# yz-cnsdqz/PSI-release

Hardware: AMD Instinct MI355X
Metric: fitting iters/sec (SMPL-X+SDF+Chamfer), PROX-E batch=32 (higher is better)
Workload: dtype f32

## Files before the change

### psi-release_amd/csrc/fit.hip

```cpp
#include "psi_internal.h"
#ifdef PSI_HEAD_STOPS
__device__ int psi_dbg_sstop;
#define PSI_SSTOP(k) do { if (psi_dbg_sstop == (k)) return; } while (0)
__device__ int psi_dbg_pstop;
#define PSI_PSTOP(k) do { if (psi_dbg_pstop == (k)) asm volatile("s_endpgm"); } while (0)
#define PSI_TRACE(lo, hi) PsiBlockTrace trace_((lo), (hi))
__device__ unsigned long long psi_dbg_tl[4 * 8192];
struct PsiBlockTrace {
    unsigned long long t0;
    int kind;
    int sel_lo, sel_hi;
    __device__ PsiBlockTrace(int lo = 9, int hi = 10) : t0(wall_clock64()), kind(0), sel_lo(lo), sel_hi(hi) {}
    __device__ ~PsiBlockTrace()
    {
        const unsigned bid = blockIdx.y * gridDim.x + blockIdx.x;
        if (psi_dbg_sstop < sel_lo || psi_dbg_sstop > sel_hi || threadIdx.x != 0 || bid >= 8192) return;
        unsigned long long *o = psi_dbg_tl + 4 * (size_t)bid;
        o[0] = t0;
        o[1] = wall_clock64();
        o[2] = (unsigned long long)__builtin_amdgcn_s_getreg((31 << 11) | 4) | ((unsigned long long)__builtin_amdgcn_s_getreg((31 << 11) | 20) << 32);
        o[3] = (unsigned long long)kind;
    }
};
extern "C" int psi_dbg_timeline(unsigned long long *out, int nblocks)
// ... 48 lines not shown
    const float *scene, *sdf, *gmin, *gmax;
    const float *sdf_brick;
    const float *Wct;
    float *x, *xhr, *cam, *adam_m, *adam_v;
    int *step;
    float *h1, *h2, *o6, *betas20, *pose, *transl, *verts, *og, *gq, *fpart, *penpart, *recpart, *vppart;
    float *cverts;
    float *g_betas, *g_pose, *g_transl, *g_rot;
    unsigned long long *hx_o6, *hx_gh1;
    unsigned *hx_epoch;
    int *hx_err;
    int hc;
#ifdef PSI_HEAD_STOPS
    int stop_h, stop_t;
#define HSTOP(k) do { if (f.stop_h == (k)) return; } while (0)
#define TSTOP(k) do { if (f.stop_t == (k)) return; } while (0)
#else
#define HSTOP(k)
#define TSTOP(k)
#endif
    int *nn_hint;
    float *history;
    int max_hist;
    int fused_bwd, ncp, ncp3;
    float *glc, *gvpc, *vpc;
    float *gtc_part;
#ifndef PSI_GV_SLOTS
#define PSI_GV_SLOTS 1024
#endif
    static_assert(PSI_GV_SLOTS >= 128, "one slot per body and class at least: fused_bwd runs batches up to 128 (merged_scene)");
    unsigned *gvbits;
    int gv_sps;
    const float *dirs_ch;
    const float *WTt_c;
    float *gA_part, *gfeat_part;
    float *spb;
    int nsv, nsv_c, nsn_m, nsn_c, spm, spc;
};

__device__ __forceinline__ float leaky(float v, float slope) { return v > 0.0f ? v : v * slope; }

__device__ __forceinline__ void gs_forward(const float *x6, float *R)
{
    float a1[3] = {x6[0], x6[2], x6[4]}, a2[3] = {x6[1], x6[3], x6[5]};
    float n1 = fmaxf(sqrtf(a1[0] * a1[0] + a1[1] * a1[1] + a1[2] * a1[2]), 1e-12f);
    float b1[3] = {a1[0] / n1, a1[1] / n1, a1[2] / n1};
    float d = b1[0] * a2[0] + b1[1] * a2[1] + b1[2] * a2[2];
    float u[3] = {a2[0] - d * b1[0], a2[1] - d * b1[1], a2[2] - d * b1[2]};
    float n2 = fmaxf(sqrtf(u[0] * u[0] + u[1] * u[1] + u[2] * u[2]), 1e-12f);
    float b2[3] = {u[0] / n2, u[1] / n2, u[2] / n2};
    float b3[3] = {b1[1] * b2[2] - b1[2] * b2[1], b1[2] * b2[0] - b1[0] * b2[2], b1[0] * b2[1] - b1[1] * b2[0]};
    for (int r = 0; r < 3; r++) {
        R[r * 3 + 0] = b1[r];
        R[r * 3 + 1] = b2[r];
        R[r * 3 + 2] = b3[r];
    }
}

__device__ __forceinline__ void gs_backward(const float *x6, const float *gR, float *g6)
{
    float a1[3] = {x6[0], x6[2], x6[4]}, a2[3] = {x6[1], x6[3], x6[5]};
    float n1 = fmaxf(sqrtf(a1[0] * a1[0] + a1[1] * a1[1] + a1[2] * a1[2]), 1e-12f);
    float b1[3] = {a1[0] / n1, a1[1] / n1, a1[2] / n1};
    float d = b1[0] * a2[0] + b1[1] * a2[1] + b1[2] * a2[2];
    float u[3] = {a2[0] - d * b1[0], a2[1] - d * b1[1], a2[2] - d * b1[2]};
    float n2 = fmaxf(sqrtf(u[0] * u[0] + u[1] * u[1] + u[2] * u[2]), 1e-12f);
    float b2[3] = {u[0] / n2, u[1] / n2, u[2] / n2};
// ... 654 lines not shown
            a2 += p[(size_t)(i + 2 * nt) * stride];
            a3 += p[(size_t)(i + 3 * nt) * stride];
        }
        for (; i < n; i += nt) a0 += p[(size_t)i * stride];
        return block_sum((a0 + a1) + (a2 + a3), red);
    };
    const float s_rec = total(f.recpart, f.B, 1);
    const float s_vp = total(f.vppart, f.B, 1);
    const float s_f = total(f.fpart, f.B * f.nfp, 1);
    const float s_pen = total(f.penpart, f.B * f.nsdfblk, 2);
    const float n_pen = total(f.penpart + 1, f.B * f.nsdfblk, 2);
    if (t == 0) {
        stats[0] = s_rec; stats[1] = s_vp; stats[2] = s_f; stats[3] = s_pen; stats[4] = n_pen; stats[5] = 0.0f;
        *f.step += 1;
    }
}

template <int MT>
__global__ __launch_bounds__(256) __attribute__((amdgpu_waves_per_eu(2, 2))) void fit_bwd_joint_kernel(
    FitDev f, LbsDev m, const float *__restrict__ g_vp, const float *__restrict__ gl, const float *__restrict__ v_posed, int n_ska, int n_blend,
    int kgroups, int nbody, float *__restrict__ stats)
{
    constexpr int SMEM_B = psi_blend_bwd_h_smem_f4<(MT + 1) / 2>();
    __shared__ f4 smem[SMEM_B > SKA_SMEM_F4 ? SMEM_B : SKA_SMEM_F4];
    const int bid = blockIdx.x;
#ifdef PSI_HEAD_STOPS
    PsiBlockTrace trace(11, 11);
    trace.kind = bid < n_ska ? (bid % (f.nsv + f.nsv_c) < f.nsv ? 0 : 1) : (bid < n_ska + n_blend ? 2 : 4);
#endif
    if (bid < n_ska) {
        const int nsl = f.nsv + f.nsv_c, sl = bid % nsl, b0 = (bid / nsl) * nbody;
        float *part = f.gA_part + (size_t)sl * f.B * PSI_JP * 16;
        if (sl < f.nsv) {
            const PsiSkaSlice o = {m.WTt + (size_t)sl * 4 * PSI_JP * 64, gl + (size_t)sl * 768, v_posed + (size_t)sl * 768, (size_t)m.Npad, part};
            skin_bwd_A_dispatch(o, f.B, b0, nbody, smem);
        } else {
            const int c = sl - f.nsv;
            const PsiSkaSlice o = {f.WTt_c + (size_t)c * 4 * PSI_JP * 64, f.glc + (size_t)c * 768, f.vpc + (size_t)c * 768, (size_t)f.ncp3, part};
            skin_bwd_A_dispatch(o, f.B, b0, nbody, smem);
        }
    } else if (bid < n_ska + n_blend) {
        int kg, slice, bg;
        psi_blend_bwd_place(bid - n_ska, kgroups, f.nsn_m + f.nsn_c, kg, slice, bg);
#ifdef PSI_HEAD_STOPS
        trace.kind = slice < f.nsn_m ? 2 : 3;
#endif
        float *part = f.gfeat_part + (size_t)slice * f.B * m.Kpad;
        const float dsc_inv = m.dirs_unscale * PSI_FEAT_SCALE;
        if (slice < f.nsn_m) {
            const PsiBlendBwdColsH o = {m.dirs_bh, g_vp, (size_t)m.Npad, m.Kpad, m.Npad / 16, f.gvbits, f.gv_sps, dsc_inv};
            blend_bwd_h_body<(MT + 1) / 2>(o, f.B, slice * f.spm, (slice + 1) * f.spm, part, kg, bg, smem);
        } else {
            const int c = slice - f.nsn_m;
            const PsiBlendBwdColsH o = {f.dirs_ch, f.gvpc, (size_t)f.ncp3, m.Kpad, f.ncp3 / 16, f.gvbits + PSI_GV_SLOTS, f.gv_sps, dsc_inv};
            blend_bwd_h_body<(MT + 1) / 2>(o, f.B, c * f.spc, (c + 1) * f.spc, part, kg, bg, smem);
        }
    } else {
        fit_stats_body(f, stats);
    }
}

__global__ __launch_bounds__(256) void fit_reduce_kernel(FitDev f, PsiLbsView lv, const float *__restrict__ stats)
{
    const int B = f.B, Kpad = lv.m.Kpad;
    const long nA = (long)B * PSI_JP * 16, nF = (long)B * Kpad, nT = (long)B * 4;
    const long t = (long)blockIdx.x * 256 + threadIdx.x;
    const long i = t / PSI_RSPL;
    const int s0 = (int)(t % PSI_RSPL);
    float spg = 0.0f;
    if (!f.indep) {
        const float N = stats[4];
// ... 15 lines not shown
        const float sp = f.indep ? f.spb[b] : spg;
        const float pen = psi_sum_slices_split<8>(f.gfeat_part + k, (size_t)nF, f.nsn_m, s0);
        const float con = psi_sum_slices_split<2>(f.gfeat_part + (size_t)f.nsn_m * nF + k, (size_t)nF, f.nsn_c, s0);
        if (s0 == 0) ((float *)lv.gfeat)[k] = __builtin_fmaf(sp, pen, con);
    } else if (i < nA + nF + nT) {
        const long k = i - nA - nF;
        const int b = (int)(k >> 2), c = (int)(k & 3), cc = c < 3 ? c : 0;
        const float sp = f.indep ? f.spb[b] : spg;
        const float pen = psi_sum_slices_split<12>(lv.gt_part + (size_t)b * 4 + cc, (size_t)B * 4, lv.nvb, s0);
        const float con = psi_sum_slices_split<8>(f.gtc_part + (size_t)b * f.nfp * 4 + cc, (size_t)4, f.nfp, s0);
        if (s0 == 0 && c < 3) f.g_transl[(size_t)b * 3 + c] = __builtin_fmaf(sp, pen, con);
    }
    if (t >= 64 && t < 64 + 2 * PSI_GV_SLOTS) f.gvbits[t - 64] = 0u;
    if (t == 0) {
        const int it = *f.step - 1;
        if (it >= 0) {
            float *h = f.history + (size_t)(it % f.max_hist) * 4;
            if (f.indep) {
                h[0] = f.w_rec * stats[0] / ((float)B * XD);
                h[1] = f.w_vp * stats[1] / ((float)B * NZ);
                h[2] = f.w_contact * stats[2] / ((float)B * f.n_c);
                h[3] = f.w_col * stats[3] / (float)B;
            } else {
                const float Bg = (float)B * (float)f.world, N = stats[4];
                h[0] = f.w_rec * stats[0] / (Bg * XD);
                h[1] = f.w_vp * stats[1] / (Bg * NZ);
                h[2] = f.w_contact * stats[2] / (Bg * f.n_c);
                h[3] = N > 0.0f ? f.w_col * stats[3] / N : 0.0f;
            }
        }
    }
}

__global__ void contact_weight_tiles_kernel(const float *__restrict__ Wct, int n_c, int ncp, float *__restrict__ WTt_c)
{
    const int i = blockIdx.x * 256 + threadIdx.x;
    if (i >= ncp * PSI_JP) return;
    const int tile = i / (PSI_JP * 64), j = (i / 64) % PSI_JP, s = tile * 64 + (i & 63);
    WTt_c[i] = s < n_c ? Wct[(size_t)s * PSI_JP + j] : 0.0f;
}
__global__ void contact_dirs_h_kernel(const float *__restrict__ dirs_bh, int Kpad, const int *__restrict__ vid, int n_c, int ncp3, float *__restrict__ dirs_ch)
{
    const size_t i = (size_t)blockIdx.x * 256 + threadIdx.x, n_all = (size_t)ncp3 * Kpad;
    if (i >= n_all) return;
    const int ne = (int)(i & 7), kr = (int)((i >> 3) & 31), nh = (int)((i >> 8) & 1), KT = Kpad / 32;
    const int kt = (int)((i >> 9) % KT), s = (int)((i >> 9) / KT);
    const int n = s * 16 + nh * 8 + ne;
    const int slot = n / 3, comp = n - 3 * slot;
    _Float16 hi = (_Float16)0.0f, lo = (_Float16)0.0f;
    if (slot < n_c) {
        const int sn = 3 * vid[slot] + comp;
        const size_t so = ((((size_t)(sn >> 4) * KT + kt) * 2) * 2 + ((sn >> 3) & 1)) * 256 + (size_t)kr * 8 + (sn & 7);
        hi = ((const _Float16 *)dirs_bh)[so];
        lo = ((const _Float16 *)dirs_bh)[so + 512];
    }
    const size_t o = ((((size_t)s * KT + kt) * 2) * 2 + nh) * 256 + (size_t)kr * 8 + ne;
    ((_Float16 *)dirs_ch)[o] = hi;
    ((_Float16 *)dirs_ch)[o + 512] = lo;
}
template <bool LOCAL>
struct FitGradSource {
    FitDev f;
    float *stats;
    float N;
    float *sNb;
    int b0;
    static constexpr int NPF = 4;
    psi_f2 pp[NPF];
    bool pp_valid;
    struct Pre { float og[3], q[3]; int cw; };
    __device__ __forceinline__ Pre issue(int b, int v, bool live)
    {
// ... 811 lines not shown
    size_t o_lws = take(lbs_floats * 4), o_nws = take(psi_nn_ws_bytes(B, f.n_c, f.m));
    hipError_t err = hipMalloc((void **)&e->blob, o);
    if (err != hipSuccess) {
        psi_set_error("psi_fit_create: hipMalloc(%zu) failed: %s", o, hipGetErrorString(err));
        return (int)err;
    }
    err = hipMemset(e->blob + zero_begin, 0, o - zero_begin);
    if (err == hipSuccess) err = hipMemset(e->blob + o_hint, 0xff, (size_t)B * f.n_c * 4);
    for (auto &it : items)
        if (err == hipSuccess) err = hipMemcpy(e->blob + it.off, it.src, it.bytes, hipMemcpyHostToDevice);
    if (err != hipSuccess) {
        psi_set_error("psi_fit_create: upload failed: %s", hipGetErrorString(err));
        return (int)err;
    }
    char *bl = e->blob;
    auto F = [&](size_t off) { return (float *)(bl + off); };
    f.W1T = F(o_w1t); f.b1 = F(o_b1); f.W2T = F(o_w2t); f.b2 = F(o_b2); f.W3T = F(o_w3t); f.b3 = F(o_b3);
    f.W1 = F(o_w1); f.W2 = F(o_w2); f.W3 = F(o_w3); f.lhc = F(o_lh); f.rhc = F(o_rh); f.pose_mean = F(o_pm);
    f.vid = (const int *)(bl + o_vid); f.cs_ptr = (const int *)(bl + o_cp); f.cs_idx = (const int *)(bl + o_ci); f.cs_first = (const int *)(bl + o_cf);
    f.gmin = F(o_gmin); f.gmax = F(o_gmax);
    f.x = F(o_x); f.xhr = F(o_xhr); f.cam = F(o_cam); f.adam_m = F(o_am); f.adam_v = F(o_av); f.step = (int *)(bl + o_step); f.hx_err = f.step + 1;
    f.h1 = F(o_h1); f.h2 = F(o_h2); f.o6 = F(o_o6); f.betas20 = F(o_b20); f.pose = F(o_pose); f.transl = F(o_tr);
    f.verts = F(o_verts); f.cverts = F(o_cv); f.og = F(o_og); f.gq = F(o_gq); f.fpart = F(o_fp); f.penpart = F(o_pp);
    f.recpart = F(o_rp); f.vppart = F(o_vp); f.g_betas = F(o_gb); f.g_pose = F(o_gp); f.g_transl = F(o_gt); f.g_rot = F(o_gr);
    f.history = F(o_hist);
    f.nn_hint = (int *)(bl + o_hint);
    f.hx_o6 = (unsigned long long *)(bl + o_hxo); f.hx_gh1 = (unsigned long long *)(bl + o_hxg); f.hx_epoch = (unsigned *)(bl + o_hxc);
    e->stats_local = F(o_stats);
    e->lbs_ws = F(o_lws);
    if (int rcv = psi_lbs_view(lbs, B, e->lbs_ws, &e->lv)) return rcv;
    e->plan = fit_plan_make(f, e->lv.m, knobs.ska_nbody);
    f.Wct = F(o_wct);
    if (e->fused_bwd) {
        f.glc = F(o_glc); f.gvpc = F(o_gvpc); f.vpc = F(o_vpc); f.gtc_part = F(o_gtc); f.WTt_c = F(o_wttc); f.dirs_ch = F(o_dirsc); f.gvbits = (unsigned *)(bl + o_gvb);
        f.gA_part = F(o_gap); f.gfeat_part = F(o_gfp); f.spb = F(o_spb);
    }
    e->skin_nb = cfg->B > 128 && !e->lv.m.Wc ? 2 : 1;
    if (knobs.skin_nb) e->skin_nb = knobs.skin_nb;
    hipLaunchKernelGGL(contact_weight_table_kernel, dim3(psi_cdiv((long)f.n_c * PSI_JP, 256)), dim3(256), 0, 0, e->lv.m.WT, e->lv.m.Vpad, f.vid,
                       f.n_c, J, (float *)f.Wct);
    if (e->fused_bwd) {
        hipLaunchKernelGGL(contact_weight_tiles_kernel, dim3(psi_cdiv((long)f.ncp * PSI_JP, 256)), dim3(256), 0, 0, f.Wct, f.n_c, f.ncp, (float *)f.WTt_c);
        hipLaunchKernelGGL(contact_dirs_h_kernel, dim3(psi_cdiv((long)f.ncp3 * e->lv.m.Kpad, 256)), dim3(256), 0, 0, e->lv.m.dirs_bh, e->lv.m.Kpad, f.vid,
                           f.n_c, f.ncp3, (float *)f.dirs_ch);
    }
    f.sdf_brick = nullptr;
    if (bricks) {
#if PSI_SDF_CELLS
        const size_t n = (size_t)f.D * f.D * f.D * 8;
        hipLaunchKernelGGL(sdf_to_cells_kernel, dim3((unsigned)psi_cdiv((long)n, 256)), dim3(256), 0, 0, d_sdf, F(o_brick), f.D);
#else
        const size_t n = (size_t)(f.D / 4) * (f.D / 4) * (f.D / 4) * PSI_BRICK_FLOATS;
        hipLaunchKernelGGL(sdf_to_bricks_kernel, dim3((unsigned)psi_cdiv((long)n, 256)), dim3(256), 0, 0, d_sdf, F(o_brick), f.D);
#endif
        f.sdf_brick = F(o_brick);
    }
    e->grid = psi_sdf_grid_make(f.sdf_brick, h_gmin, h_gmax, f.D, f.align_corners);
    err = hipDeviceSynchronize();
    if (err == hipSuccess) err = hipGetLastError();
    if (err != hipSuccess) {
        psi_set_error("psi_fit_create: layout kernels failed: %s", hipGetErrorString(err));
        return (int)err;
    }
    e->nn_ws = bl + o_nws;
    if (cfg->nn_mode == 1) {
        std::vector<float> hs((size_t)f.m * 3);
        err = hipMemcpy(hs.data(), d_scene_verts, hs.size() * 4, hipMemcpyDeviceToHost);
        if (int rc = err == hipSuccess ? psi_nn_index_create(&e->nn_index, hs.data(), f.m) : (int)err) return rc;
    }
    owner.release();
    *out = e;
    return 0;
}

extern "C" void psi_fit_destroy(psi_fit_engine *e)
// ... 269 lines not shown
```

### psi-release_amd/csrc/lbs.hip

```cpp
#include "psi_internal.h"
#include "lbs_device.h"
#include <algorithm>
#include <math.h>
#include <stdlib.h>
#include <vector>
#include <string.h>

typedef float f4 __attribute__((ext_vector_type(4)));
typedef float f2 __attribute__((ext_vector_type(2)));

namespace {

constexpr int JP = PSI_JP;
constexpr int SKIN_BLK = PSI_SKIN_BLK;

}

struct psi_lbs_model {
    LbsDev d;
    void *blob;
};

namespace {

// ... 172 lines not shown
    float mx = 0.0f;
    for (int i = p * 256 + (int)threadIdx.x; i < npad4; i += P * 256) {
        const f4 v = row[i];
        mx = fmaxf(mx, fmaxf(fmaxf(fabsf(v[0]), fabsf(v[1])), fmaxf(fabsf(v[2]), fabsf(v[3]))));
    }
#pragma unroll
    for (int o2 = 32; o2 > 0; o2 >>= 1) mx = fmaxf(mx, __shfl_xor(mx, o2, 64));
    if ((threadIdx.x & 63) == 0) red[threadIdx.x >> 6] = mx;
    __syncthreads();
    if (threadIdx.x == 0) slots[(size_t)b * P + p] = __float_as_uint(fmaxf(fmaxf(red[0], red[1]), fmaxf(red[2], red[3])));
}

template <int MT>
__global__ __launch_bounds__(256) __attribute__((amdgpu_waves_per_eu(2, 2))) void bwd_joint_kernel(
    LbsDev m, const float *__restrict__ g_vp, const float *__restrict__ gl, const float *__restrict__ v_posed, int B, int steps_per_slice,
    float *__restrict__ gfeat_part, float *__restrict__ gA_part, int n_blend, int kgroups, int nslices, int nsv, int nbody,
    const unsigned *__restrict__ gvbits, int gvparts)
{
    constexpr int SMEM_B = psi_blend_bwd_h_smem_f4<(MT + 1) / 2>();
    __shared__ f4 smem[SMEM_B > SKA_SMEM_F4 ? SMEM_B : SKA_SMEM_F4];
    const int n_ska = (int)gridDim.x - n_blend;
    const int bid = (int)blockIdx.x >= n_ska ? (int)blockIdx.x - n_ska : (int)blockIdx.x + n_blend;
#ifdef PSI_HEAD_STOPS
    PsiBlockTrace2 trace;
    trace.kind = bid < n_blend;
#endif
    if (bid < n_blend) {
        int kg, slice, bg;
        psi_blend_bwd_place(bid, kgroups, nslices, kg, slice, bg);
        const PsiBlendBwdColsH cols = {m.dirs_bh, g_vp, (size_t)m.Npad, m.Kpad, m.Npad / 16, gvbits, gvparts, m.dirs_unscale * PSI_FEAT_SCALE};
        blend_bwd_h_body<(MT + 1) / 2>(cols, B, slice * steps_per_slice, (slice + 1) * steps_per_slice, gfeat_part + (size_t)slice * B * m.Kpad, kg, bg, smem);
    } else {
        const int i = bid - n_blend, vslice = i % nsv;
        const PsiSkaSlice sl = {m.WTt + (size_t)vslice * 4 * PSI_JP * 64, gl + (size_t)vslice * 768, v_posed + (size_t)vslice * 768, (size_t)m.Npad,
                                gA_part + (size_t)vslice * B * JP * 16};
        skin_bwd_A_dispatch(sl, B, (i / nsv) * nbody, nbody, smem);
    }
}

constexpr int RSPL = PSI_RSPL;
__global__ __launch_bounds__(256) void reduce_partials_kernel(int B, int Kpad, const float *__restrict__ gA_part, int nsv,
                                                              const float *__restrict__ gfeat_part, int nsn,
                                                              const float *__restrict__ gt_part, int nvb,
                                                              float *__restrict__ gA, float *__restrict__ gfeat,
                                                              float *__restrict__ g_transl)
{
    const long nA = (long)B * JP * 16, nF = (long)B * Kpad, nT = (long)B * 4;
    const long t = (long)blockIdx.x * 256 + threadIdx.x;
    const long i = t / RSPL;
    const int s0 = (int)(t % RSPL);
    if (i < nA) {
        const float r = (i & 15) < 12 ? psi_sum_slices_split<12>(gA_part + i, (size_t)nA, nsv, s0) : 0.0f;
        if (s0 == 0) gA[i] = r;
    } else if (i < nA + nF) {
        const long k = i - nA;
        const float r = psi_sum_slices_split<8>(gfeat_part + k, (size_t)nF, nsn, s0);
        if (s0 == 0) gfeat[k] = r;
    } else if (i < nA + nF + nT) {
        const long k = i - nA - nF;
        const int b = (int)(k >> 2), c = (int)(k & 3);
        const float r = psi_sum_slices_split<12>(gt_part + (size_t)b * 4 + (c < 3 ? c : 0), (size_t)B * 4, nvb, s0);
        if (s0 == 0 && c < 3 && g_transl) g_transl[(size_t)b * 3 + c] = r;
    }
}

__global__ __launch_bounds__(256) void pose_bwd_kernel(LbsDev m, const float *__restrict__ betas, const float *__restrict__ pose,
                                                      const float *__restrict__ Rs, const float *__restrict__ Jls,
// ... 87 lines not shown
        if (amax > 0.0f) (void)std::frexp(amax, &e);
        const float scale = std::ldexp(1.0f, 14 - e);
        d.dirs_unscale = 1.0f / (scale * PSI_FEAT_SCALE);
        _Float16 *dh = reinterpret_cast<_Float16 *>(dirs.data());
        for (int k = 0; k < d.Kpad; k++)
            for (int n = 0; n < d.Npad; n++) {
                const float x = dirs_at(k, n) * scale;
                const _Float16 hi = (_Float16)x;
                const _Float16 lo = (_Float16)((x - (float)hi) * 2048.0f);
                const size_t o = (size_t)(n >> 5) * d.dirs_tile * 2 + ((size_t)(k >> 4) * 4 + ((k >> 3) & 1)) * 256 + (size_t)(n & 31) * 8 + (k & 7);
                dh[o] = hi;
                dh[o + 512] = lo;
            }
        dirs_bh.assign((size_t)d.Kpad * d.Npad, 0.0f);
        _Float16 *bh = reinterpret_cast<_Float16 *>(dirs_bh.data());
        const int KT = d.Kpad / 32;
        for (int k = 0; k < d.Kpad; k++)
            for (int n = 0; n < d.Npad; n++) {
                const float x = dirs_at(k, n) * scale;
                const _Float16 hi = (_Float16)x;
                const _Float16 lo = (_Float16)((x - (float)hi) * 2048.0f);
                const size_t o = ((((size_t)(n >> 4) * KT + (k >> 5)) * 2) * 2 + ((n >> 3) & 1)) * 256 + (size_t)(k & 31) * 8 + (n & 7);
                bh[o] = hi;
                bh[o + 512] = lo;
            }
    }
    memcpy(vt.data(), h_v_template, sizeof(float) * d.N);
    std::vector<float> WTt((size_t)JP * d.Vpad, 0.0f);
    for (int v = 0; v < V; v++)
        for (int j = 0; j < J; j++) {
            WT[(size_t)j * d.Vpad + v] = h_weights[(size_t)v * J + j];
            WTt[((size_t)(v >> 6) * JP + j) * 64 + (v & 63)] = h_weights[(size_t)v * J + j];
        }
    std::vector<float> Jt((size_t)J * 3), Js((size_t)J * 3 * (NB > 0 ? NB : 1), 0.0f);
    {
        std::vector<double> acc((size_t)3 * (NB + 1));
        for (int j = 0; j < J; j++) {
            std::fill(acc.begin(), acc.end(), 0.0);
            const float *jr = h_J_regressor + (size_t)j * V;
            for (int v = 0; v < V; v++) {
                double wv = jr[v];
                if (wv == 0.0) continue;
                for (int c = 0; c < 3; c++) {
                    acc[c * (NB + 1) + NB] += wv * h_v_template[(size_t)v * 3 + c];
                    const float *sd = h_shapedirs + ((size_t)v * 3 + c) * NB;
                    for (int l = 0; l < NB; l++) acc[c * (NB + 1) + l] += wv * sd[l];
                }
            }
            for (int c = 0; c < 3; c++) {
                Jt[j * 3 + c] = (float)acc[c * (NB + 1) + NB];
                for (int l = 0; l < NB; l++) Js[((size_t)j * 3 + c) * NB + l] = (float)acc[c * (NB + 1) + l];
            }
        }
    }
    std::vector<float> Wc;
    std::vector<unsigned> Wj;
    {
        int nnz_max = 0;
        for (int v = 0; v < V; v++) {
            int c = 0;
            for (int j = 0; j < J; j++) c += h_weights[(size_t)v * J + j] != 0.0f;
            nnz_max = std::max(nnz_max, c);
        }
        const char *dense = getenv("PSI_LBS_DENSE");
        if (nnz_max <= PSI_WNZ && !(dense && dense[0] == '1')) {
            Wc.assign((size_t)PSI_WNZ * d.Vpad, 0.0f);
            Wj.assign((size_t)(PSI_WNZ / 4) * d.Vpad, 0u);
            for (int v = 0; v < V; v++) {
                int k = 0;
                for (int j = 0; j < J; j++) {
                    float w = h_weights[(size_t)v * J + j];
                    if (w != 0.0f) { Wc[(size_t)k * d.Vpad + v] = w; Wj[(size_t)(k >> 2) * d.Vpad + v] |= (unsigned)j << (8 * (k & 3)); k++; }
                }
            }
        }
    }
    size_t o = 0;
    auto take = [&](size_t bytes) { size_t r = o; o += (bytes + 255) & ~(size_t)255; return r; };
    size_t o_dirs = take(dirs.size() * 4), o_dirs_bh = take(dirs_bh.size() * 4), o_vt = take(vt.size() * 4), o_wt = take(WT.size() * 4), o_wtt = take(WTt.size() * 4), o_jt = take(Jt.size() * 4),
           o_js = take(Js.size() * 4), o_wc = take(Wc.size() * 4 + 4), o_wj = take(Wj.size() * 4 + 4), o_par = take(J * 4), o_lvl = take(J * 4), o_cp = take((J + 1) * 4), o_ci = take(cidx.size() * 4),
           o_jump = take(jump.size() * 4), o_sl = take(sub_list.size()), o_si = take(sub_item.size() * 4), o_sf = take(sub_first.size());
    char *blob = nullptr;
    PSI_CHECK_HIP(hipMalloc((void **)&blob, o));
    std::vector<int> par(h_parents, h_parents + J);
    struct { size_t off; const void *src; size_t bytes; } cp[] = {
        {o_dirs, dirs.data(), dirs.size() * 4}, {o_dirs_bh, dirs_bh.data(), dirs_bh.size() * 4}, {o_vt, vt.data(), vt.size() * 4}, {o_wt, WT.data(), WT.size() * 4}, {o_wtt, WTt.data(), WTt.size() * 4},
        {o_jt, Jt.data(), Jt.size() * 4}, {o_js, Js.data(), Js.size() * 4}, {o_wc, Wc.data(), Wc.size() * 4}, {o_wj, Wj.data(), Wj.size() * 4},
        {o_par, par.data(), (size_t)J * 4},
        {o_lvl, level.data(), (size_t)J * 4}, {o_cp, cptr.data(), (size_t)(J + 1) * 4}, {o_ci, cidx.data(), cidx.size() * 4},
        {o_jump, jump.data(), jump.size() * 4}, {o_sl, sub_list.data(), sub_list.size()}, {o_si, sub_item.data(), sub_item.size() * 4},
        {o_sf, sub_first.data(), sub_first.size()}};
    for (auto &c : cp) {
        if (!c.bytes) continue;
        hipError_t e = hipMemcpy(blob + c.off, c.src, c.bytes, hipMemcpyHostToDevice);
        if (e != hipSuccess) {
            (void)hipFree(blob);
            psi_set_error("hipMemcpy failed: %s", hipGetErrorString(e));
            return (int)e;
        }
    }
    d.dirs = (const float *)(blob + o_dirs);
    d.dirs_bh = (const float *)(blob + o_dirs_bh);
    d.v_template = (const float *)(blob + o_vt);
    d.WT = (const float *)(blob + o_wt);
    d.WTt = (const float *)(blob + o_wtt);
    d.Wc = Wc.empty() ? nullptr : (const float *)(blob + o_wc);
    d.Wj = Wj.empty() ? nullptr : (const unsigned *)(blob + o_wj);
    d.J_t = (const float *)(blob + o_jt);
    d.J_s = (const float *)(blob + o_js);
    d.parents = (const int *)(blob + o_par);
    d.level = (const int *)(blob + o_lvl);
    d.child_ptr = (const int *)(blob + o_cp);
    d.child_idx = (const int *)(blob + o_ci);
    d.jump = (const int *)(blob + o_jump);
    d.sub_list = (const unsigned char *)(blob + o_sl);
    d.sub_item = (const unsigned int *)(blob + o_si);
    d.sub_first = (const unsigned char *)(blob + o_sf);
    psi_lbs_model *mdl = new psi_lbs_model;
    mdl->d = d;
    mdl->blob = blob;
    *out = mdl;
    return 0;
}

extern "C" void psi_lbs_destroy(psi_lbs_model *m)
{
    if (!m) return;
    (void)hipFree(m->blob);
    delete m;
}

extern "C" size_t psi_lbs_workspace_floats(const psi_lbs_model *m, int B)
{
    if (!m || B <= 0) return 0;
    return ws_layout(m->d, B).total;
}

static int lbs_launch_blend(const LbsDev &m, const WsLayout &L, int B, float *ws, hipStream_t st)
// ... 166 lines not shown
```

### psi-release_amd/csrc/lbs_device.h

```cpp
#pragma once
#ifndef PSI_TRACE
#define PSI_TRACE(lo, hi)
#endif
#ifndef PSI_SSTOP
#define PSI_SSTOP(k)
#endif
#ifndef PSI_PSTOP
#define PSI_PSTOP(k)
#endif
#include <hip/hip_runtime.h>

typedef float psi_f4 __attribute__((ext_vector_type(4)));

constexpr int PSI_JP = 64;
constexpr int PSI_SUB_MAX = PSI_JP * (PSI_JP + 1) / 2;
constexpr int PSI_ITEM_MAX = 2 * PSI_JP;
constexpr int PSI_NJUMP = 6;
constexpr int PSI_WNZ = 8;
constexpr int PSI_A_TAIL = 16;

struct LbsDev {
    int V, J, NB, P, K, Kpad, N, Npad, Vpad, maxlevel, njump;
    int dirs_tile;
    float dirs_unscale;
    const float *dirs, *v_template, *WT, *J_t, *J_s;
    const float *dirs_bh;
    const float *WTt;
    const float *Wc;
    const unsigned *Wj;
    const int *parents, *level, *child_ptr, *child_idx;
    const int *jump;
    const unsigned char *sub_list;
    const unsigned int *sub_item;
    const unsigned char *sub_first;
    int n_sub, n_items;
};

struct PsiLbsView {
    LbsDev m;
    float *feat, *R, *Jl, *G, *A, *v_posed, *gl, *g_vp, *gt_part_w;
    const float *gA_part, *gfeat_part, *gt_part;
    const float *gA, *gfeat;
    int nsv, nsn, nvb;
};

__device__ __forceinline__ void psi_rodrigues(const float *aa, float *R)
{
    float x = aa[0] + 1e-8f, y = aa[1] + 1e-8f, z = aa[2] + 1e-8f;
    float angle = sqrtf(x * x + y * y + z * z);
    float rx = aa[0] / angle, ry = aa[1] / angle, rz = aa[2] / angle;
    float s = sinf(angle), c1 = 1.0f - cosf(angle);
    R[0] = 1.0f + c1 * (-(ry * ry + rz * rz));
    R[1] = s * (-rz) + c1 * (rx * ry);
    R[2] = s * ry + c1 * (rx * rz);
    R[3] = s * rz + c1 * (rx * ry);
    R[4] = 1.0f + c1 * (-(rx * rx + rz * rz));
    R[5] = s * (-rx) + c1 * (ry * rz);
    R[6] = s * (-ry) + c1 * (rx * rz);
    R[7] = s * rx + c1 * (ry * rz);
    R[8] = 1.0f + c1 * (-(rx * rx + ry * ry));
// ... 894 lines not shown
```

### psi-release_amd/csrc/lbs_joint_device.h

```cpp
#pragma once
#include "lbs_device.h"

#ifndef PSI_SKA_MARK
#define PSI_SKA_MARK(k)
#endif

constexpr int SKA_NBODY = 8;
constexpr int SKA_ROW = 256 + 16;
constexpr int SKA_MAXT = (12 * SKA_NBODY + 15) / 16;
constexpr int SKA_SMEM_F4 = SKA_NBODY * 2 * 3 * SKA_ROW / 4;

struct PsiSkaSlice {
    const float *wtt;
    const float *gl, *vp;
    size_t row_stride;
    float *part;
};

template <int NT>
__device__ __forceinline__ void skin_bwd_A_body(const PsiSkaSlice &o, int B, int b0, int nbody, psi_f4 *smem)
{
    typedef psi_f4 f4;
    const int lane = threadIdx.x & 63, w = threadIdx.x >> 6;
    const int li = lane & 15, lk = lane >> 4;
    const int nb = min(nbody, B - b0);
    const int ncol = 12 * nb;
    f4 wa[16];
    {
        const f4 *wr = (const f4 *)(o.wtt + ((size_t)lk * PSI_JP + (w * 16 + li)) * 64);
#pragma unroll
        for (int q = 0; q < 16; q++) wa[q] = wr[q];
    }
    float *sG = (float *)smem;
    float *sP = sG + SKA_NBODY * 3 * SKA_ROW;
    {
        f4 og[SKA_NBODY], op[SKA_NBODY];
        const int t4 = threadIdx.x;
#pragma unroll
        for (int bb = 0; bb < SKA_NBODY; bb++)
            if (bb < nb && t4 < 192) {
                og[bb] = *(const f4 *)(o.gl + (size_t)(b0 + bb) * o.row_stride + t4 * 4);
                op[bb] = *(const f4 *)(o.vp + (size_t)(b0 + bb) * o.row_stride + t4 * 4);
            }
#pragma unroll
        for (int bb = 0; bb < SKA_NBODY; bb++)
            if (bb < nb && t4 < 192) {
#pragma unroll
                for (int e = 0; e < 4; e++) {
                    const int i = t4 * 4 + e, v = i / 3, comp = i - 3 * v;
                    const int pos = (bb * 3 + comp) * SKA_ROW + v + 4 * (v >> 6);
                    sG[pos] = og[bb][e];
                    sP[pos] = op[bb][e];
                }
            }
    }
    __syncthreads();
    PSI_SKA_MARK(0);
    int goff[NT], poff[NT];
    f4 acc[NT];
#pragma unroll
    for (int nt = 0; nt < NT; nt++) {
        const int c = min(16 * nt + li, ncol - 1);
        const int bb = c / 12, rs = c - 12 * bb, r = rs >> 2, sx = rs & 3;
        goff[nt] = (bb * 3 + r) * SKA_ROW + lk * 68;
        poff[nt] = sx < 3 ? (bb * 3 + sx) * SKA_ROW + lk * 68 : -1;
        acc[nt] = (f4){0, 0, 0, 0};
    }
#pragma unroll
    for (int q = 0; q < 16; q++) {
        f4 bop[NT];
#pragma unroll
        for (int nt = 0; nt < NT; nt++) {
            const f4 g4 = *(const f4 *)(sG + goff[nt] + 4 * q);
            const f4 p4 = *(const f4 *)(sP + max(poff[nt], 0) + 4 * q);
            bop[nt] = poff[nt] >= 0 ? g4 * p4 : g4;
        }
#pragma unroll
        for (int e = 0; e < 4; e++)
#pragma unroll
            for (int nt = 0; nt < NT; nt++) acc[nt] = __builtin_amdgcn_mfma_f32_16x16x4f32(wa[q][e], bop[nt][e], acc[nt], 0, 0, 0);
        if (q == 0) PSI_SKA_MARK(1);
        __builtin_amdgcn_sched_barrier(0);
    }
#pragma unroll
    for (int nt = 0; nt < NT; nt++) {
        const int c = 16 * nt + li;
        if (c < ncol) {
            const int bb = c / 12, rs = c - 12 * bb;
            float *po = o.part + (((size_t)(b0 + bb)) * PSI_JP + w * 16 + lk * 4) * 16 + rs;
#pragma unroll
            for (int e = 0; e < 4; e++) po[e * 16] = acc[nt][e];
        }
    }
}

__device__ __forceinline__ void skin_bwd_A_dispatch(const PsiSkaSlice &o, int B, int b0, int nbody, psi_f4 *smem)
{
    switch ((12 * nbody + 15) >> 4) {
    case 1: skin_bwd_A_body<1>(o, B, b0, nbody, smem); break;
    case 2: skin_bwd_A_body<2>(o, B, b0, nbody, smem); break;
    case 3: skin_bwd_A_body<3>(o, B, b0, nbody, smem); break;
    case 4: skin_bwd_A_body<4>(o, B, b0, nbody, smem); break;
    case 5: skin_bwd_A_body<5>(o, B, b0, nbody, smem); break;
    default: skin_bwd_A_body<SKA_MAXT>(o, B, b0, nbody, smem); break;
    }
}

typedef _Float16 psi_h8 __attribute__((ext_vector_type(8)));
typedef float psi_f16v __attribute__((ext_vector_type(16)));
typedef unsigned int psi_u4 __attribute__((ext_vector_type(4)));
struct PsiBlendBwdColsH {
    const float *dirs_bh;
    const float *g_vp;
    size_t row_stride;
    int Kpad, total_steps;
    const unsigned *gvbits;
    int gv_slots;
    float dsc_inv;
};
__device__ __forceinline__ float psi_fp16_row_scale(unsigned bits)
{
    int E = (int)((bits >> 23) & 0xffu);
    if (bits == 0u) E = 140;
    int se = 267 - E;
    se = se < 27 ? 27 : (se > 227 ? 227 : se);
    return __uint_as_float((unsigned)se << 23);
}
template <int MTB>
constexpr int psi_blend_bwd_h_smem_f4() { return 4 * 2 * MTB * 4 * 64; }

template <int MTB>
__device__ __forceinline__ void blend_bwd_h_body(const PsiBlendBwdColsH &o, int B, int s_begin, int s_end, float *__restrict__ part, int kgroup,
                                                 int bgroup, psi_f4 *smem)
{
    typedef psi_f4 f4;
    const int lane = threadIdx.x & 63, w = threadIdx.x >> 6;
    const int li = lane & 31, kh = lane >> 5;
    const int KT = o.Kpad / 32;
    const int k0 = kgroup * 64;
    const int b0 = bgroup * 32 * MTB;
    s_end = min(s_end, o.total_steps);
    psi_f16v acc[2][MTB][2];
#pragma unroll
    for (int kt = 0; kt < 2; kt++)
#pragma unroll
        for (int t = 0; t < MTB; t++)
#pragma unroll
            for (int c = 0; c < 2; c++)
#pragma unroll
                for (int i = 0; i < 16; i++) acc[kt][t][c][i] = 0.0f;
    const float *grow[MTB];
#pragma unroll
    for (int t = 0; t < MTB; t++) grow[t] = o.g_vp + (size_t)min(b0 + t * 32 + li, B - 1) * o.row_stride + 8 * kh;
    const char *dbase = (const char *)o.dirs_bh + ((size_t)(2 * kgroup) * 2) * 1024 + (size_t)(kh * 32 + li) * 16;
    float gsc[MTB], us[MTB];
#pragma unroll
    for (int t = 0; t < MTB; t++) {
        const unsigned *sl = o.gvbits + (size_t)min(b0 + t * 32 + li, B - 1) * o.gv_slots;
        unsigned cbits = 0u;
        for (int p = kh; p < o.gv_slots; p += 2) cbits = max(cbits, sl[p]);
// ... 89 lines not shown
```

Baseline: 10380.

## Switch skinning-weight backward to split-fp16 32x32 MFMA with scaled operands

Replaces the fp32 16x16x4 MFMA path in the skinning A-gradient backward with fp16 32x32x16 MFMAs. Both weights and the per-body scaled products are split into hi and lo halves and combined with three MFMAs to keep near-fp32 accuracy. Weights are pre-packed on the host (and for contact vertices by a setup kernel) into a new fp16 hi/lo layout. Each wave now covers half of the vertex range, and partial sums are exchanged through shared memory. The aim is higher matrix throughput and fewer MFMA issues per column, at the cost of a per-body scale reduction, an extra sync and exchange, and some precision risk.

```diff
diff --git a/psi-release_amd/csrc/fit.hip b/psi-release_amd/csrc/fit.hip
--- a/psi-release_amd/csrc/fit.hip
+++ b/psi-release_amd/csrc/fit.hip
@@ -104,7 +104,7 @@
     unsigned *gvbits;
     int gv_sps;
     const float *dirs_ch;
-    const float *WTt_c;
+    const float *WTh_c;
     float *gA_part, *gfeat_part;
     float *spb;
     int nsv, nsv_c, nsn_m, nsn_c, spm, spc;
@@ -825,11 +825,11 @@
         const int nsl = f.nsv + f.nsv_c, sl = bid % nsl, b0 = (bid / nsl) * nbody;
         float *part = f.gA_part + (size_t)sl * f.B * PSI_JP * 16;
         if (sl < f.nsv) {
-            const PsiSkaSlice o = {m.WTt + (size_t)sl * 4 * PSI_JP * 64, gl + (size_t)sl * 768, v_posed + (size_t)sl * 768, (size_t)m.Npad, part};
+            const PsiSkaSlice o = {m.WTh + (size_t)sl * 4 * PSI_JP * 64, gl + (size_t)sl * 768, v_posed + (size_t)sl * 768, (size_t)m.Npad, part};
             skin_bwd_A_dispatch(o, f.B, b0, nbody, smem);
         } else {
             const int c = sl - f.nsv;
-            const PsiSkaSlice o = {f.WTt_c + (size_t)c * 4 * PSI_JP * 64, f.glc + (size_t)c * 768, f.vpc + (size_t)c * 768, (size_t)f.ncp3, part};
+            const PsiSkaSlice o = {f.WTh_c + (size_t)c * 4 * PSI_JP * 64, f.glc + (size_t)c * 768, f.vpc + (size_t)c * 768, (size_t)f.ncp3, part};
             skin_bwd_A_dispatch(o, f.B, b0, nbody, smem);
         }
     } else if (bid < n_ska + n_blend) {
@@ -911,12 +911,16 @@
     }
 }
 
-__global__ void contact_weight_tiles_kernel(const float *__restrict__ Wct, int n_c, int ncp, float *__restrict__ WTt_c)
+__global__ void contact_weight_parts_kernel(const float *__restrict__ Wct, int n_c, int ncp, float *__restrict__ WTh_c)
 {
     const int i = blockIdx.x * 256 + threadIdx.x;
     if (i >= ncp * PSI_JP) return;
-    const int tile = i / (PSI_JP * 64), j = (i / 64) % PSI_JP, s = tile * 64 + (i & 63);
-    WTt_c[i] = s < n_c ? Wct[(size_t)s * PSI_JP + j] : 0.0f;
+    const int s = i / PSI_JP, j = i - s * PSI_JP;
+    const float x = s < n_c ? Wct[i] : 0.0f;
+    const _Float16 hi = (_Float16)x;
+    const size_t o = psi_ska_wth_index(s, j);
+    ((_Float16 *)WTh_c)[o] = hi;
+    ((_Float16 *)WTh_c)[o + 512] = (_Float16)((x - (float)hi) * 2048.0f);
 }
 __global__ void contact_dirs_h_kernel(const float *__restrict__ dirs_bh, int Kpad, const int *__restrict__ vid, int n_c, int ncp3, float *__restrict__ dirs_ch)
 {
@@ -1794,7 +1798,7 @@
     e->plan = fit_plan_make(f, e->lv.m, knobs.ska_nbody);
     f.Wct = F(o_wct);
     if (e->fused_bwd) {
-        f.glc = F(o_glc); f.gvpc = F(o_gvpc); f.vpc = F(o_vpc); f.gtc_part = F(o_gtc); f.WTt_c = F(o_wttc); f.dirs_ch = F(o_dirsc); f.gvbits = (unsigned *)(bl + o_gvb);
+        f.glc = F(o_glc); f.gvpc = F(o_gvpc); f.vpc = F(o_vpc); f.gtc_part = F(o_gtc); f.WTh_c = F(o_wttc); f.dirs_ch = F(o_dirsc); f.gvbits = (unsigned *)(bl + o_gvb);
         f.gA_part = F(o_gap); f.gfeat_part = F(o_gfp); f.spb = F(o_spb);
     }
     e->skin_nb = cfg->B > 128 && !e->lv.m.Wc ? 2 : 1;
@@ -1802,7 +1806,7 @@
     hipLaunchKernelGGL(contact_weight_table_kernel, dim3(psi_cdiv((long)f.n_c * PSI_JP, 256)), dim3(256), 0, 0, e->lv.m.WT, e->lv.m.Vpad, f.vid,
                        f.n_c, J, (float *)f.Wct);
     if (e->fused_bwd) {
-        hipLaunchKernelGGL(contact_weight_tiles_kernel, dim3(psi_cdiv((long)f.ncp * PSI_JP, 256)), dim3(256), 0, 0, f.Wct, f.n_c, f.ncp, (float *)f.WTt_c);
+        hipLaunchKernelGGL(contact_weight_parts_kernel, dim3(psi_cdiv((long)f.ncp * PSI_JP, 256)), dim3(256), 0, 0, f.Wct, f.n_c, f.ncp, (float *)f.WTh_c);
         hipLaunchKernelGGL(contact_dirs_h_kernel, dim3(psi_cdiv((long)f.ncp3 * e->lv.m.Kpad, 256)), dim3(256), 0, 0, e->lv.m.dirs_bh, e->lv.m.Kpad, f.vid,
                            f.n_c, f.ncp3, (float *)f.dirs_ch);
     }
diff --git a/psi-release_amd/csrc/lbs.hip b/psi-release_amd/csrc/lbs.hip
--- a/psi-release_amd/csrc/lbs.hip
+++ b/psi-release_amd/csrc/lbs.hip
@@ -228,7 +228,7 @@
         blend_bwd_h_body<(MT + 1) / 2>(cols, B, slice * steps_per_slice, (slice + 1) * steps_per_slice, gfeat_part + (size_t)slice * B * m.Kpad, kg, bg, smem);
     } else {
         const int i = bid - n_blend, vslice = i % nsv;
-        const PsiSkaSlice sl = {m.WTt + (size_t)vslice * 4 * PSI_JP * 64, gl + (size_t)vslice * 768, v_posed + (size_t)vslice * 768, (size_t)m.Npad,
+        const PsiSkaSlice sl = {m.WTh + (size_t)vslice * 4 * PSI_JP * 64, gl + (size_t)vslice * 768, v_posed + (size_t)vslice * 768, (size_t)m.Npad,
                                 gA_part + (size_t)vslice * B * JP * 16};
         skin_bwd_A_dispatch(sl, B, (i / nsv) * nbody, nbody, smem);
     }
@@ -382,6 +382,18 @@
             WT[(size_t)j * d.Vpad + v] = h_weights[(size_t)v * J + j];
             WTt[((size_t)(v >> 6) * JP + j) * 64 + (v & 63)] = h_weights[(size_t)v * J + j];
         }
+    std::vector<float> WTh((size_t)JP * d.Vpad, 0.0f);
+    {
+        _Float16 *wh = reinterpret_cast<_Float16 *>(WTh.data());
+        for (int v = 0; v < V; v++)
+            for (int j = 0; j < J; j++) {
+                const float x = h_weights[(size_t)v * J + j];
+                const _Float16 hi = (_Float16)x;
+                const size_t o = psi_ska_wth_index(v, j);
+                wh[o] = hi;
+                wh[o + 512] = (_Float16)((x - (float)hi) * 2048.0f);
+            }
+    }
     std::vector<float> Jt((size_t)J * 3), Js((size_t)J * 3 * (NB > 0 ? NB : 1), 0.0f);
     {
         std::vector<double> acc((size_t)3 * (NB + 1));
@@ -427,7 +439,7 @@
     }
     size_t o = 0;
     auto take = [&](size_t bytes) { size_t r = o; o += (bytes + 255) & ~(size_t)255; return r; };
-    size_t o_dirs = take(dirs.size() * 4), o_dirs_bh = take(dirs_bh.size() * 4), o_vt = take(vt.size() * 4), o_wt = take(WT.size() * 4), o_wtt = take(WTt.size() * 4), o_jt = take(Jt.size() * 4),
+    size_t o_dirs = take(dirs.size() * 4), o_dirs_bh = take(dirs_bh.size() * 4), o_vt = take(vt.size() * 4), o_wt = take(WT.size() * 4), o_wtt = take(WTt.size() * 4), o_wth = take(WTh.size() * 4), o_jt = take(Jt.size() * 4),
            o_js = take(Js.size() * 4), o_wc = take(Wc.size() * 4 + 4), o_wj = take(Wj.size() * 4 + 4), o_par = take(J * 4), o_lvl = take(J * 4), o_cp = take((J + 1) * 4), o_ci = take(cidx.size() * 4),
            o_jump = take(jump.size() * 4), o_sl = take(sub_list.size()), o_si = take(sub_item.size() * 4), o_sf = take(sub_first.size());
     char *blob = nullptr;
@@ -435,6 +447,7 @@
     std::vector<int> par(h_parents, h_parents + J);
     struct { size_t off; const void *src; size_t bytes; } cp[] = {
         {o_dirs, dirs.data(), dirs.size() * 4}, {o_dirs_bh, dirs_bh.data(), dirs_bh.size() * 4}, {o_vt, vt.data(), vt.size() * 4}, {o_wt, WT.data(), WT.size() * 4}, {o_wtt, WTt.data(), WTt.size() * 4},
+        {o_wth, WTh.data(), WTh.size() * 4},
         {o_jt, Jt.data(), Jt.size() * 4}, {o_js, Js.data(), Js.size() * 4}, {o_wc, Wc.data(), Wc.size() * 4}, {o_wj, Wj.data(), Wj.size() * 4},
         {o_par, par.data(), (size_t)J * 4},
         {o_lvl, level.data(), (size_t)J * 4}, {o_cp, cptr.data(), (size_t)(J + 1) * 4}, {o_ci, cidx.data(), cidx.size() * 4},
@@ -454,6 +467,7 @@
     d.v_template = (const float *)(blob + o_vt);
     d.WT = (const float *)(blob + o_wt);
     d.WTt = (const float *)(blob + o_wtt);
+    d.WTh = (const float *)(blob + o_wth);
     d.Wc = Wc.empty() ? nullptr : (const float *)(blob + o_wc);
     d.Wj = Wj.empty() ? nullptr : (const unsigned *)(blob + o_wj);
     d.J_t = (const float *)(blob + o_jt);
diff --git a/psi-release_amd/csrc/lbs_device.h b/psi-release_amd/csrc/lbs_device.h
--- a/psi-release_amd/csrc/lbs_device.h
+++ b/psi-release_amd/csrc/lbs_device.h
@@ -26,6 +26,7 @@
     const float *dirs, *v_template, *WT, *J_t, *J_s;
     const float *dirs_bh;
     const float *WTt;
+    const float *WTh;
     const float *Wc;
     const unsigned *Wj;
     const int *parents, *level, *child_ptr, *child_idx;
diff --git a/psi-release_amd/csrc/lbs_joint_device.h b/psi-release_amd/csrc/lbs_joint_device.h
--- a/psi-release_amd/csrc/lbs_joint_device.h
+++ b/psi-release_amd/csrc/lbs_joint_device.h
@@ -7,32 +7,63 @@
 
 constexpr int SKA_NBODY = 8;
 constexpr int SKA_ROW = 256 + 16;
-constexpr int SKA_MAXT = (12 * SKA_NBODY + 15) / 16;
-constexpr int SKA_SMEM_F4 = SKA_NBODY * 2 * 3 * SKA_ROW / 4;
+constexpr int SKA_MAXT = (12 * SKA_NBODY + 31) / 32;
+constexpr int SKA_ROWS = SKA_NBODY * 2 * 3 + 1;
+constexpr int SKA_SMEM_F4 = (SKA_ROWS * SKA_ROW + SKA_NBODY) / 4;
+static_assert(4 * SKA_MAXT * 2 * 64 <= SKA_ROWS * SKA_ROW / 4, "the waves' exchange of half tiles reuses the staged rows");
+
+__host__ __device__ inline size_t psi_ska_wth_index(int v, int j)
+{
+    const int sl = v >> 8, vh = (v >> 7) & 1, ks = (v >> 4) & 7, kh = (v >> 3) & 1, e = v & 7;
+    const int wv = (j >> 5) + 2 * vh, lane = kh * 32 + (j & 31);
+    return ((((size_t)sl * 4 + wv) * 8 + ks) * 2 * 64 + lane) * 8 + e;
+}
+
+typedef _Float16 psi_h8 __attribute__((ext_vector_type(8)));
+typedef float psi_f16v __attribute__((ext_vector_type(16)));
+typedef unsigned int psi_u4 __attribute__((ext_vector_type(4)));
+
+__device__ __forceinline__ float psi_fp16_row_scale(unsigned bits)
+{
+    int E = (int)((bits >> 23) & 0xffu);
+    if (bits == 0u) E = 140;
+    int se = 267 - E;
+    se = se < 27 ? 27 : (se > 227 ? 227 : se);
+    return __uint_as_float((unsigned)se << 23);
+}
 
 struct PsiSkaSlice {
-    const float *wtt;
+    const float *wth;
     const float *gl, *vp;
     size_t row_stride;
     float *part;
 };
 
+#ifndef PSI_SKA_AHEAD
+#define PSI_SKA_AHEAD 1
+#endif
+
 template <int NT>
 __device__ __forceinline__ void skin_bwd_A_body(const PsiSkaSlice &o, int B, int b0, int nbody, psi_f4 *smem)
 {
     typedef psi_f4 f4;
     const int lane = threadIdx.x & 63, w = threadIdx.x >> 6;
-    const int li = lane & 15, lk = lane >> 4;
+    const int li = lane & 31, kh = lane >> 5;
+    const int jt = w & 1, vh = w >> 1;
     const int nb = min(nbody, B - b0);
     const int ncol = 12 * nb;
-    f4 wa[16];
+    psi_u4 wa[8][2];
     {
-        const f4 *wr = (const f4 *)(o.wtt + ((size_t)lk * PSI_JP + (w * 16 + li)) * 64);
-#pragma unroll
-        for (int q = 0; q < 16; q++) wa[q] = wr[q];
+        const psi_u4 *wr = (const psi_u4 *)o.wth + (size_t)w * 16 * 64 + lane;
+#pragma unroll
+        for (int ks = 0; ks < 8; ks++)
+#pragma unroll
+            for (int p = 0; p < 2; p++) wa[ks][p] = wr[(ks * 2 + p) * 64];
     }
     float *sG = (float *)smem;
     float *sP = sG + SKA_NBODY * 3 * SKA_ROW;
+    float *sOne = sP + SKA_NBODY * 3 * SKA_ROW;
+    float *sS = sOne + SKA_ROW;
     {
         f4 og[SKA_NBODY], op[SKA_NBODY];
         const int t4 = threadIdx.x;
@@ -42,6 +73,8 @@
                 og[bb] = *(const f4 *)(o.gl + (size_t)(b0 + bb) * o.row_stride + t4 * 4);
                 op[bb] = *(const f4 *)(o.vp + (size_t)(b0 + bb) * o.row_stride + t4 * 4);
             }
+        if (t4 >= 192)
+            for (int i = t4 - 192; i < SKA_ROW / 4; i += 64) ((f4 *)sOne)[i] = (f4){1.0f, 1.0f, 1.0f, 1.0f};
 #pragma unroll
         for (int bb = 0; bb < SKA_NBODY; bb++)
             if (bb < nb && t4 < 192) {
@@ -55,60 +88,124 @@
             }
     }
     __syncthreads();
+    {
+        const int bb = threadIdx.x >> 5, j = threadIdx.x & 31;
+        unsigned mg = 0u, mp = 0u;
+        if (bb < nb) {
+            const int pos = bb * 3 * SKA_ROW + 8 * j + 4 * (j >> 3);
+#pragma unroll
+            for (int c = 0; c < 3; c++)
+#pragma unroll
+                for (int h = 0; h < 2; h++) {
+                    const psi_u4 a = *(const psi_u4 *)(sG + pos + c * SKA_ROW + 4 * h) & 0x7fffffffu;
+                    const psi_u4 b = *(const psi_u4 *)(sP + pos + c * SKA_ROW + 4 * h) & 0x7fffffffu;
+                    mg = max(max(mg, max(a[0], a[1])), max(a[2], a[3]));
+                    mp = max(max(mp, max(b[0], b[1])), max(b[2], b[3]));
+                }
+        }
+#pragma unroll
+        for (int o2 = 16; o2 > 0; o2 >>= 1) {
+            mg = max(mg, (unsigned)__shfl_xor((int)mg, o2, 64));
+            mp = max(mp, (unsigned)__shfl_xor((int)mp, o2, 64));
+        }
+        if (j == 0 && bb < nb) {
+            const float M = __uint_as_float(mg) * fmaxf(1.0f, __uint_as_float(mp));
+            sS[bb] = psi_fp16_row_scale(__float_as_uint(M) & 0x7fffffffu);
+        }
+    }
+    __syncthreads();
     PSI_SKA_MARK(0);
     int goff[NT], poff[NT];
-    f4 acc[NT];
+    float sc[NT];
+    psi_f16v acc[NT][2];
 #pragma unroll
     for (int nt = 0; nt < NT; nt++) {
-        const int c = min(16 * nt + li, ncol - 1);
+        const int c = min(32 * nt + li, ncol - 1);
         const int bb = c / 12, rs = c - 12 * bb, r = rs >> 2, sx = rs & 3;
-        goff[nt] = (bb * 3 + r) * SKA_ROW + lk * 68;
-        poff[nt] = sx < 3 ? (bb * 3 + sx) * SKA_ROW + lk * 68 : -1;
-        acc[nt] = (f4){0, 0, 0, 0};
-    }
-#pragma unroll
-    for (int q = 0; q < 16; q++) {
-        f4 bop[NT];
-#pragma unroll
-        for (int nt = 0; nt < NT; nt++) {
-            const f4 g4 = *(const f4 *)(sG + goff[nt] + 4 * q);
-            const f4 p4 = *(const f4 *)(sP + max(poff[nt], 0) + 4 * q);
-            bop[nt] = poff[nt] >= 0 ? g4 * p4 : g4;
-        }
-#pragma unroll
-        for (int e = 0; e < 4; e++)
-#pragma unroll
-            for (int nt = 0; nt < NT; nt++) acc[nt] = __builtin_amdgcn_mfma_f32_16x16x4f32(wa[q][e], bop[nt][e], acc[nt], 0, 0, 0);
-        if (q == 0) PSI_SKA_MARK(1);
+        const int base = 136 * vh + 8 * kh;
+        goff[nt] = (bb * 3 + r) * SKA_ROW + base;
+        poff[nt] = (sx < 3 ? (SKA_NBODY * 3 + bb * 3 + sx) * SKA_ROW : SKA_NBODY * 6 * SKA_ROW) + base;
+        sc[nt] = sS[bb];
+#pragma unroll
+        for (int c2 = 0; c2 < 2; c2++)
+#pragma unroll
+            for (int i = 0; i < 16; i++) acc[nt][c2][i] = 0.0f;
+    }
+    f4 cur[4], nxt[4];
+    auto request = [&](int t, f4 (&d)[4]) {
+        const int ks = t / NT, nt = t - ks * NT, off = 16 * ks + 4 * (ks >> 2);
+        d[0] = *(const f4 *)(sG + goff[nt] + off);
+        d[1] = *(const f4 *)(sG + goff[nt] + off + 4);
+        d[2] = *(const f4 *)(sG + poff[nt] + off);
+        d[3] = *(const f4 *)(sG + poff[nt] + off + 4);
+    };
+    if (PSI_SKA_AHEAD) request(0, cur);
+#pragma unroll
+    for (int t = 0; t < 8 * NT; t++) {
+        const int ks = t / NT, nt = t - ks * NT;
+        if (!PSI_SKA_AHEAD) request(t, cur);
+        else if (t + 1 < 8 * NT) request(t + 1, nxt);
+        psi_h8 ph, pl;
+#pragma unroll
+        for (int e = 0; e < 8; e++) {
+            const float x = cur[e >> 2][e & 3] * cur[2 + (e >> 2)][e & 3] * sc[nt];
+            const _Float16 hi = (_Float16)x;
+            ph[e] = hi;
+            pl[e] = (_Float16)((x - (float)hi) * 2048.0f);
+        }
+        const psi_h8 wh = __builtin_bit_cast(psi_h8, wa[ks][0]), wl = __builtin_bit_cast(psi_h8, wa[ks][1]);
+        acc[nt][1] = __builtin_amdgcn_mfma_f32_32x32x16_f16(wh, pl, acc[nt][1], 0, 0, 0);
+        acc[nt][0] = __builtin_amdgcn_mfma_f32_32x32x16_f16(wh, ph, acc[nt][0], 0, 0, 0);
+        acc[nt][1] = __builtin_amdgcn_mfma_f32_32x32x16_f16(wl, ph, acc[nt][1], 0, 0, 0);
+        if (PSI_SKA_AHEAD && t + 1 < 8 * NT) {
+#pragma unroll
+            for (int i = 0; i < 4; i++) cur[i] = nxt[i];
+        }
+        if (t == 0) PSI_SKA_MARK(1);
         __builtin_amdgcn_sched_barrier(0);
     }
+    f4 v[NT][4];
 #pragma unroll
     for (int nt = 0; nt < NT; nt++) {
-        const int c = 16 * nt + li;
+        const float us = 1.0f / sc[nt], us2 = us * (1.0f / 2048.0f);
+#pragma unroll
+        for (int q = 0; q < 4; q++)
+#pragma unroll
+            for (int e = 0; e < 4; e++) v[nt][q][e] = __builtin_fmaf(acc[nt][1][4 * q + e], us2, acc[nt][0][4 * q + e] * us);
+    }
+    __syncthreads();
+    f4 (*xc)[NT][2][64] = (f4 (*)[NT][2][64])smem;
+#pragma unroll
+    for (int nt = 0; nt < NT; nt++)
+#pragma unroll
+        for (int qq = 0; qq < 2; qq++) xc[w][nt][qq][lane] = vh ? v[nt][2 * qq] : v[nt][2 * qq + 1];
+    __syncthreads();
+#pragma unroll
+    for (int nt = 0; nt < NT; nt++) {
+        const int c = 32 * nt + li;
         if (c < ncol) {
             const int bb = c / 12, rs = c - 12 * bb;
-            float *po = o.part + (((size_t)(b0 + bb)) * PSI_JP + w * 16 + lk * 4) * 16 + rs;
-#pragma unroll
-            for (int e = 0; e < 4; e++) po[e * 16] = acc[nt][e];
+#pragma unroll
+            for (int qq = 0; qq < 2; qq++) {
+                const f4 mine = vh ? v[nt][2 * qq + 1] : v[nt][2 * qq], theirs = xc[w ^ 2][nt][qq][lane];
+                const f4 sum = vh ? theirs + mine : mine + theirs;
+                float *po = o.part + (((size_t)(b0 + bb)) * PSI_JP + 32 * jt + 8 * (2 * qq + vh) + 4 * kh) * 16 + rs;
+#pragma unroll
+                for (int e = 0; e < 4; e++) po[e * 16] = sum[e];
+            }
         }
     }
 }
 
 __device__ __forceinline__ void skin_bwd_A_dispatch(const PsiSkaSlice &o, int B, int b0, int nbody, psi_f4 *smem)
 {
-    switch ((12 * nbody + 15) >> 4) {
+    switch ((12 * nbody + 31) >> 5) {
     case 1: skin_bwd_A_body<1>(o, B, b0, nbody, smem); break;
     case 2: skin_bwd_A_body<2>(o, B, b0, nbody, smem); break;
-    case 3: skin_bwd_A_body<3>(o, B, b0, nbody, smem); break;
-    case 4: skin_bwd_A_body<4>(o, B, b0, nbody, smem); break;
-    case 5: skin_bwd_A_body<5>(o, B, b0, nbody, smem); break;
     default: skin_bwd_A_body<SKA_MAXT>(o, B, b0, nbody, smem); break;
     }
 }
 
-typedef _Float16 psi_h8 __attribute__((ext_vector_type(8)));
-typedef float psi_f16v __attribute__((ext_vector_type(16)));
-typedef unsigned int psi_u4 __attribute__((ext_vector_type(4)));
 struct PsiBlendBwdColsH {
     const float *dirs_bh;
     const float *g_vp;
@@ -118,14 +215,6 @@
     int gv_slots;
     float dsc_inv;
 };
-__device__ __forceinline__ float psi_fp16_row_scale(unsigned bits)
-{
-    int E = (int)((bits >> 23) & 0xffu);
-    if (bits == 0u) E = 140;
-    int se = 267 - E;
-    se = se < 27 ? 27 : (se > 227 ? 227 : se);
-    return __uint_as_float((unsigned)se << 23);
-}
 template <int MTB>
 constexpr int psi_blend_bwd_h_smem_f4() { return 4 * 2 * MTB * 4 * 64; }
 
```

Result: no change. 10430 (median of 3 runs) (+0.5%).
